# GiorgiaAuroraAdorni/gansformer-reproducibility-challenge

Hardware: NVIDIA H100
Metric: images/sec @256^2 synth (GANsformer generator forward, K=16 latents, 12 attention layers, batch 32/GPU) (higher is better)
Workload: dtype tf32 (fp32 storage; wgmma tf32 attention and stride-1 3x3 convolutions (own kernels), TF32 cuDNN up-convolutions; value_fp32_convs = the same with fp32 cuDNN convolutions)

## Files before the change

### gansformer-reproducibility-challenge_b200/_build.py

```python
from __future__ import annotations

import os
import shutil
import subprocess
from pathlib import Path

PKG_DIR = Path(__file__).resolve().parent
CSRC = PKG_DIR / "csrc"
LIB_PATH = PKG_DIR / "libgf_attn.so"
SOURCES = ["gf_api.cu", "gf_fold.cu", "gf_simt.cu", "gf_tc.cu", "gf_tc_cen.cu", "gf_tc_gemm.cu", "gf_bwd.cu", "gf_ops.cu", "gf_conv.cu"]
COMPILE_FLAGS = [
    "-gencode", "arch=compute_90a,code=sm_90a",
    "-lineinfo", "-O3", "-std=c++17",
    "-Xcompiler", "-fPIC",
]


def _nvcc() -> str:
    for cand in (os.environ.get("NVCC"), shutil.which("nvcc"), "/usr/local/cuda/bin/nvcc"):
        if cand and os.path.exists(cand):
            return cand
    raise RuntimeError("nvcc not found: cannot build libgf_attn.so (set NVCC=/path/to/nvcc)")


def _stale() -> bool:
    if not LIB_PATH.exists():
        return True
    t = LIB_PATH.stat().st_mtime
    deps = list(CSRC.glob("*.cu")) + list(CSRC.glob("*.cuh")) + list((PKG_DIR.parent / "include").glob("*.h"))
    return any(d.stat().st_mtime > t for d in deps)


def _compile_one(nvcc: str, src: Path, obj: Path, verbose: bool) -> str:
    cmd = [nvcc, *COMPILE_FLAGS, *os.environ.get("GF_NVCC_DEFS", "").split(), "-c", str(src), "-o", str(obj)]
    if verbose:
        cmd[1:1] = ["-Xptxas", "-v"]
    res = subprocess.run(cmd, capture_output=True, text=True)
    if res.returncode != 0:
        raise RuntimeError("nvcc failed:\n" + " ".join(cmd) + "\n" + res.stdout + res.stderr)
    return res.stderr


def build_extension(force: bool = False, verbose: bool = False) -> Path:
    if not force and not _stale():
        return LIB_PATH
    from concurrent.futures import ThreadPoolExecutor
    nvcc = _nvcc()
    objdir = PKG_DIR / "build"
    objdir.mkdir(exist_ok=True)
    tag = objdir / ".flags"
    flags_now = " ".join(COMPILE_FLAGS) + "|" + os.environ.get("GF_NVCC_DEFS", "")
    if not tag.exists() or tag.read_text() != flags_now:
        force = True
    hdr_time = max(d.stat().st_mtime for d in list(CSRC.glob("*.cuh")) + list((PKG_DIR.parent / "include").glob("*.h")))
    jobs = []
    for name in SOURCES:
        src, obj = CSRC / name, objdir / (name[:-3] + ".o")
        if force or verbose or not obj.exists() or obj.stat().st_mtime < max(src.stat().st_mtime, hdr_time):
            jobs.append((src, obj))
    with ThreadPoolExecutor(max_workers=min(8, max(1, len(jobs)))) as pool:
        logs = list(pool.map(lambda j: _compile_one(nvcc, j[0], j[1], verbose), jobs))
    tag.write_text(flags_now)
    cmd = [nvcc, "-gencode", "arch=compute_90a,code=sm_90a", "-shared", "-o", str(LIB_PATH)] + [str(objdir / (n[:-3] + ".o")) for n in SOURCES]
    res = subprocess.run(cmd, capture_output=True, text=True)
    if res.returncode != 0:
        raise RuntimeError("nvcc link failed:\n" + " ".join(cmd) + "\n" + res.stdout + res.stderr)
    if verbose:
        print("\n".join(logs))
    return LIB_PATH
```

### gansformer-reproducibility-challenge_b200/csrc/gf_conv.cu

```cuda
#include <stdlib.h>
#include <string.h>
#include "gf_common.cuh"
#include "gf_tc_common.cuh"
#include "../../include/gf_ops.h"

namespace gf {
namespace cv {

using namespace tc;

constexpr int PH = 8, PW = 16;
constexpr int BK = 32;
constexpr int A_ROWS = (PH + 2) * PW;
constexpr int A_BYTES = A_ROWS * BK * 4;
constexpr int NUM_THREADS = 288;
constexpr int MAX_A = 3, MAX_W = 8;

struct Bars {
  uint64_t full_a[MAX_A], empty_a[MAX_A], full_w[MAX_W], empty_w[MAX_W];
};

struct Params {
  int B, H, W, Cin, Cout;
  int tiles_h, tiles_w, tiles_n;
  long long total_tiles;
  int na, nw;
  float alpha;
};

__device__ __forceinline__ void tma_load_4d(uint32_t dst, const CUtensorMap* map, uint32_t bar, int c0, int c1, int c2, int c3) {
  asm volatile(
      "cp.async.bulk.tensor.4d.shared::cluster.global.mbarrier::complete_tx::bytes [%0], [%1, {%3, %4, %5, %6}], [%2];"
      ::"r"(dst), "l"(map), "r"(bar), "r"(c0), "r"(c1), "r"(c2), "r"(c3)
      : "memory");
}

template <int BN>
__global__ void __launch_bounds__(NUM_THREADS, 1)
conv3x3_tc_kernel(const __grid_constant__ CUtensorMap tmX, const __grid_constant__ CUtensorMap tmW, float* __restrict__ y, const Params P) {
  constexpr int W_BYTES = BN * BK * 4;
  extern __shared__ __align__(1024) uint8_t smem_raw[];
  uint8_t* smem = smem_raw + ((1024u - (smem_u32(smem_raw) & 1023u)) & 1023u);
  const uint32_t s_a = smem_u32(smem);
  const uint32_t s_w = s_a + (uint32_t)P.na * A_BYTES;
  Bars* bars = reinterpret_cast<Bars*>(smem + (size_t)P.na * A_BYTES + (size_t)P.nw * W_BYTES);
  const int warp = __shfl_sync(0xffffffffu, (int)(threadIdx.x >> 5), 0);
  const int lane = threadIdx.x & 31;

  if (warp == 8 && lane == 0) {
    prefetch_tmap(&tmX); prefetch_tmap(&tmW);
    for (int i = 0; i < P.na; ++i) { mbar_init(smem_u32(&bars->full_a[i]), 1); mbar_init(smem_u32(&bars->empty_a[i]), 2); }
    for (int i = 0; i < P.nw; ++i) { mbar_init(smem_u32(&bars->full_w[i]), 1); mbar_init(smem_u32(&bars->empty_w[i]), 2); }
    fence_barrier_init();
  }
  __syncthreads();

  auto decode = [&](long long t, int& nt, int& pw, int& ph, int& b) {
    nt = (int)(t % P.tiles_n); t /= P.tiles_n;
    pw = (int)(t % P.tiles_w); t /= P.tiles_w;
    ph = (int)(t % P.tiles_h); b = (int)(t / P.tiles_h);
  };

  if (warp == 8) {
    if (lane == 0) {
      int sa = 0, sw = 0; uint32_t pa = 0, pw_ = 0;
      for (long long t = blockIdx.x; t < P.total_tiles; t += gridDim.x) {
        int nt, pw, ph, b;
        decode(t, nt, pw, ph, b);
        const int h0 = ph * PH, w0 = pw * PW, n0 = nt * BN;
        for (int c0 = 0; c0 < P.Cin; c0 += BK) {
          for (int dx = 0; dx < 3; ++dx) {
            mbar_wait(smem_u32(&bars->empty_a[sa]), pa ^ 1u);
            const uint32_t fa = smem_u32(&bars->full_a[sa]);
            mbar_expect_tx(fa, (uint32_t)A_BYTES);
            tma_load_4d(s_a + (uint32_t)sa * A_BYTES, &tmX, fa, c0, w0 + dx - 1, h0 - 1, b);
            if (++sa == P.na) { sa = 0; pa ^= 1u; }
            for (int dy = 0; dy < 3; ++dy) {
              mbar_wait(smem_u32(&bars->empty_w[sw]), pw_ ^ 1u);
              const uint32_t fw = smem_u32(&bars->full_w[sw]);
              mbar_expect_tx(fw, (uint32_t)W_BYTES);
              tma_load_2d(s_w + (uint32_t)sw * W_BYTES, &tmW, fw, c0, (dy * 3 + dx) * P.Cout + n0);
              if (++sw == P.nw) { sw = 0; pw_ ^= 1u; }
            }
          }
        }
      }
    }
    return;
  }

  const int wg = warp >> 2;
  const int gid = lane >> 2, qd = lane & 3;
  const int rA = wg * 64 + (warp & 3) * 16 + gid;
  const bool leader = (warp & 3) == 0 && lane == 0;
  int sa = 0, sw = 0; uint32_t pa = 0, pw_ = 0;
  for (long long t = blockIdx.x; t < P.total_tiles; t += gridDim.x) {
    int nt, pw, ph, b;
    decode(t, nt, pw, ph, b);
    float acc[BN / 2];
    int prev_w = -1, prev_a = -1;
#pragma unroll 1
    for (int c0 = 0; c0 < P.Cin; c0 += BK) {
#pragma unroll 1
      for (int dx = 0; dx < 3; ++dx) {
        mbar_wait(smem_u32(&bars->full_a[sa]), pa);
        const uint32_t a_view = s_a + (uint32_t)sa * A_BYTES + wg * 64 * 128;
#pragma unroll
        for (int dy = 0; dy < 3; ++dy) {
          mbar_wait(smem_u32(&bars->full_w[sw]), pw_);
          const uint64_t da = gmma_desc(a_view + dy * PW * 128, 1024, LAYOUT_SW128);
          const uint64_t db = gmma_desc(s_w + (uint32_t)sw * W_BYTES, 1024, LAYOUT_SW128);
          const uint32_t acc0 = (c0 | dx | dy) ? 1u : 0u;
          wgmma_fence();
#pragma unroll
          for (int kk = 0; kk < 4; ++kk) wgmma_ss<BN>(acc, da + kk * 2, db + kk * 2, (acc0 | kk) ? 1u : 0u);
          wgmma_commit();
          wgmma_wait<1>();
          if (prev_w >= 0) {
            named_bar_sync(1 + wg, 128);
            if (leader) {
              mbar_arrive(smem_u32(&bars->empty_w[prev_w]));
              if (prev_a >= 0) mbar_arrive(smem_u32(&bars->empty_a[prev_a]));
            }
          }
          prev_w = sw;
          prev_a = dy == 2 ? sa : -1;
          if (++sw == P.nw) { sw = 0; pw_ ^= 1u; }
        }
        if (++sa == P.na) { sa = 0; pa ^= 1u; }
      }
    }
    wgmma_wait<0>();
    fence_regs<BN / 2>(acc);
    named_bar_sync(1 + wg, 128);
    if (leader) {
      mbar_arrive(smem_u32(&bars->empty_w[prev_w]));
      mbar_arrive(smem_u32(&bars->empty_a[prev_a]));
    }
#pragma unroll
    for (int i = 0; i < 2; ++i) {
      const int r = rA + 8 * i;
      const int h = ph * PH + (r >> 4), w = pw * PW + (r & 15);
      float* yrow = y + (((size_t)b * P.H + h) * P.W + w) * P.Cout + nt * BN + 2 * qd;
#pragma unroll
      for (int j = 0; j < BN / 8; ++j)
        *reinterpret_cast<float2*>(yrow + 8 * j) = make_float2(acc[4 * j + 2 * i] * P.alpha, acc[4 * j + 2 * i + 1] * P.alpha);
    }
  }
}

constexpr int U_PC = 16, U_PR = 8;
constexpr int U_OC = U_PC - 2;
constexpr int U_BN = 64;
constexpr int U_A_BYTES = (U_PR + 1) * U_PC * BK * 4;
constexpr int U_W_BYTES = U_BN * BK * 4;
constexpr int U_WS_BYTES = 9 * U_W_BYTES;
constexpr int U_CS = 68;
constexpr int U_NA = 4;
constexpr int U_THREADS = 384;

struct UBars {
  uint64_t full_a[U_NA], empty_a[U_NA], full_w[4], empty_w[4];
};

struct UParams {
  int B, H, W, Cin, Cout;
  int strips, steps, tiles_n;
  int total_units;
  float ag;
  const float* scale;
};

__device__ constexpr int U_GTAPS[4] = {4, 2, 2, 1};
__device__ constexpr int U_GNX[4] = {2, 2, 1, 1};
__device__ constexpr int U_GTAP[4][4] = {{8, 7, 5, 4}, {2, 1, 0, 0}, {6, 3, 0, 0}, {0, 0, 0, 0}};
__device__ constexpr int U_GOFF[4] = {0, 4, 6, 8};
__device__ constexpr int U_GROW[4] = {0, 1, 0, 1};

__device__ __forceinline__ void setmaxnreg_dec40() { asm volatile("setmaxnreg.dec.sync.aligned.u32 40;"); }
__device__ __forceinline__ void setmaxnreg_inc232() { asm volatile("setmaxnreg.inc.sync.aligned.u32 232;"); }

__global__ void __launch_bounds__(U_THREADS, 1)
upconv_blur_tc_kernel(const __grid_constant__ CUtensorMap tmX, const __grid_constant__ CUtensorMap tmW, float* __restrict__ y, const UParams P) {
  extern __shared__ __align__(1024) uint8_t smem_raw[];
  uint8_t* smem = smem_raw + ((1024u - (smem_u32(smem_raw) & 1023u)) & 1023u);
  const uint32_t s_a = smem_u32(smem);
  const uint32_t s_w = s_a + (uint32_t)U_NA * U_A_BYTES;
  float* carry = reinterpret_cast<float*>(smem + (size_t)U_NA * U_A_BYTES + U_WS_BYTES);
  float* stage = carry + 4 * 2 * U_PC * U_CS;
  UBars* bars = reinterpret_cast<UBars*>(stage + U_PR * U_PC * U_CS);
  const int warp = __shfl_sync(0xffffffffu, (int)(threadIdx.x >> 5), 0);
  const int lane = threadIdx.x & 31;

  if (warp == 8 && lane == 0) {
    prefetch_tmap(&tmX); prefetch_tmap(&tmW);
    for (int i = 0; i < U_NA; ++i) { mbar_init(smem_u32(&bars->full_a[i]), 1); mbar_init(smem_u32(&bars->empty_a[i]), 2); }
    for (int i = 0; i < 4; ++i) { mbar_init(smem_u32(&bars->full_w[i]), 1); mbar_init(smem_u32(&bars->empty_w[i]), 2); }
    fence_barrier_init();
  }
  __syncthreads();

  auto decode = [&](int u, int& nt, int& st, int& b) {
    nt = u % P.tiles_n; u /= P.tiles_n;
    st = u % P.strips; b = u / P.strips;
  };

  if (warp >= 8) {
    setmaxnreg_dec40();
    if (warp == 8 && lane == 0) {
      int sa = 0; uint32_t pa = 0, pw_ = 0;
      for (int u = blockIdx.x; u < P.total_units; u += gridDim.x) {
        int nt, st, b;
        decode(u, nt, st, b);
        const int j0 = st * U_OC, n0 = nt * U_BN;
        for (int s = 0; s < P.steps; ++s) {
          for (int c0 = 0; c0 < P.Cin; c0 += BK) {
            for (int g = 0; g < 4; ++g) {
              if (g == 0 || g == 2) {
                mbar_wait(smem_u32(&bars->empty_a[sa]), pa ^ 1u);
                const uint32_t fa = smem_u32(&bars->full_a[sa]);
                mbar_expect_tx(fa, (uint32_t)U_A_BYTES);
                tma_load_4d(s_a + (uint32_t)sa * U_A_BYTES, &tmX, fa, c0, j0 - (g == 0), s * U_PR - 1, b);
                if (++sa == U_NA) { sa = 0; pa ^= 1u; }
              }
              mbar_wait(smem_u32(&bars->empty_w[g]), pw_ ^ 1u);
              const uint32_t fw = smem_u32(&bars->full_w[g]);
              mbar_expect_tx(fw, (uint32_t)(U_GTAPS[g] * U_W_BYTES));
              for (int k = 0; k < U_GTAPS[g]; ++k)
                tma_load_2d(s_w + (uint32_t)(U_GOFF[g] + k) * U_W_BYTES, &tmW, fw, c0, U_GTAP[g][k] * P.Cout + n0);
            }
            pw_ ^= 1u;
          }
        }
      }
    }
    return;
  }

  setmaxnreg_inc232();
  const int wg = warp >> 2;
  const int gid = lane >> 2, qd = lane & 3;
  const bool leader = (warp & 3) == 0 && lane == 0;
  const int cp = lane & 7, cg = lane >> 3;
  int sa = 0; uint32_t pa = 0, pw_ = 0;
  for (int u = blockIdx.x; u < P.total_units; u += gridDim.x) {
    int nt, st, b;
    decode(u, nt, st, b);
    const int j0 = st * U_OC, n0 = nt * U_BN;
    for (int s = 0; s < P.steps; ++s) {
      float accx[U_BN], accy[U_BN];
      int prev_a = -1;
      uint32_t a_view = 0;
#pragma unroll 1
      for (int c0 = 0; c0 < P.Cin; c0 += BK) {
#pragma unroll
        for (int g = 0; g < 4; ++g) {
          if (g == 0 || g == 2) {
            mbar_wait(smem_u32(&bars->full_a[sa]), pa);
            a_view = s_a + (uint32_t)sa * U_A_BYTES + wg * 4 * U_PC * 128;
          }
          mbar_wait(smem_u32(&bars->full_w[g]), pw_);
          const uint64_t da = gmma_desc(a_view + U_GROW[g] * U_PC * 128, 1024, LAYOUT_SW128);
          const uint64_t db = gmma_desc(s_w + (uint32_t)U_GOFF[g] * U_W_BYTES, 1024, LAYOUT_SW128);
          const uint64_t dby = db + (uint64_t)(U_GNX[g] * U_W_BYTES >> 4);
          const int ny = U_GTAPS[g] - U_GNX[g];
          const uint32_t acc0 = (c0 > 0 || g > 0) ? 1u : 0u;
          wgmma_fence();
#pragma unroll
          for (int kk = 0; kk < 4; ++kk) {
            const uint32_t ac = (acc0 | kk) ? 1u : 0u;
            if (U_GNX[g] == 2) wgmma_ss<128>(accx, da + kk * 2, db + kk * 2, ac);
            else wgmma_ss<64>(accx, da + kk * 2, db + kk * 2, ac);
            if (ny == 2) wgmma_ss<128>(accy, da + kk * 2, dby + kk * 2, ac);
            else if (ny == 1) wgmma_ss<64>(accy, da + kk * 2, dby + kk * 2, ac);
          }
          wgmma_commit();
          wgmma_wait<1>();
          if (c0 > 0 || g > 0) {
            named_bar_sync(1 + wg, 128);
            if (leader) {
              mbar_arrive(smem_u32(&bars->empty_w[(g + 3) & 3]));
              if (prev_a >= 0) mbar_arrive(smem_u32(&bars->empty_a[prev_a]));
            }
          }
          prev_a = (g == 1 || g == 3) ? sa : -1;
          if (g == 1 || g == 3) { if (++sa == U_NA) { sa = 0; pa ^= 1u; } }
        }
        pw_ ^= 1u;
      }
      wgmma_wait<0>();
      fence_regs<U_BN>(accx);
      fence_regs<U_BN>(accy);
      named_bar_sync(1 + wg, 128);
      if (leader) {
        mbar_arrive(smem_u32(&bars->empty_w[3]));
        mbar_arrive(smem_u32(&bars->empty_a[prev_a]));
      }

      const int io = s * U_PR - 2 + warp;
#pragma unroll
      for (int sl = 0; sl < U_BN / 16; ++sl) {
        float* my_row = stage + warp * U_PC * U_CS;
#pragma unroll
        for (int ph = 0; ph < 4; ++ph)
#pragma unroll
          for (int jj = 0; jj < 2; ++jj)
#pragma unroll
            for (int i = 0; i < 2; ++i)
              *reinterpret_cast<float2*>(my_row + (gid + 8 * i) * U_CS + ph * 16 + jj * 8 + 2 * qd) =
                  make_float2((ph < 2 ? accx : accy)[32 * (ph & 1) + 4 * (2 * sl + jj) + 2 * i], (ph < 2 ? accx : accy)[32 * (ph & 1) + 4 * (2 * sl + jj) + 2 * i + 1]);
        named_bar_sync(3, 256);
        if (io >= 0 && io < P.H) {
          auto row = [&](int r) -> const float* {
            return (r < 2 ? carry + (sl * 2 + r) * U_PC * U_CS : stage + (r - 2) * U_PC * U_CS) + 2 * cp;
          };
          const int ch = n0 + sl * 16 + 2 * cp;
          const float2 d = __ldg(reinterpret_cast<const float2*>(P.scale + (size_t)b * P.Cout + ch));
          const float2 f = make_float2(P.ag * d.x, P.ag * d.y);
          const int Wo = 2 * P.W;
#pragma unroll 1
          for (int p = cg; p < U_OC && j0 + p < P.W; p += 4) {
            float* y0 = y + (((size_t)b * 2 * P.H + 2 * io) * Wo + 2 * (j0 + p)) * P.Cout + ch;
            float2 e0, o0, e1, o1;
#pragma unroll
            for (int v = 0; v < 5; ++v) {
              const float* base = row(warp + v / 2) + ((v & 1) ? 0 : 32) + p * U_CS;
              const float2 E0 = *reinterpret_cast<const float2*>(base), O0 = *reinterpret_cast<const float2*>(base + 16);
              const float2 E1 = *reinterpret_cast<const float2*>(base + U_CS), O1 = *reinterpret_cast<const float2*>(base + U_CS + 16);
              const float2 O2 = *reinterpret_cast<const float2*>(base + 2 * U_CS + 16);
              float2 h0, h1;
              h0.x = ((O0.x + 3.f * E0.x) + 3.f * O1.x) + E1.x;
              h0.y = ((O0.y + 3.f * E0.y) + 3.f * O1.y) + E1.y;
              h1.x = ((E0.x + 3.f * O1.x) + 3.f * E1.x) + O2.x;
              h1.y = ((E0.y + 3.f * O1.y) + 3.f * E1.y) + O2.y;
              if (v == 0) { e0 = h0; e1 = h1; }
              else if (v == 1) {
                e0.x += 3.f * h0.x; e0.y += 3.f * h0.y; o0 = h0;
                e1.x += 3.f * h1.x; e1.y += 3.f * h1.y; o1 = h1;
              } else if (v == 2) {
                e0.x += 3.f * h0.x; e0.y += 3.f * h0.y; o0.x += 3.f * h0.x; o0.y += 3.f * h0.y;
                e1.x += 3.f * h1.x; e1.y += 3.f * h1.y; o1.x += 3.f * h1.x; o1.y += 3.f * h1.y;
              } else if (v == 3) {
                e0.x += h0.x; e0.y += h0.y; o0.x += 3.f * h0.x; o0.y += 3.f * h0.y;
                e1.x += h1.x; e1.y += h1.y; o1.x += 3.f * h1.x; o1.y += 3.f * h1.y;
              } else {
                o0.x += h0.x; o0.y += h0.y;
                o1.x += h1.x; o1.y += h1.y;
              }
            }
            *reinterpret_cast<float2*>(y0) = make_float2(e0.x * 0.015625f * f.x, e0.y * 0.015625f * f.y);
            *reinterpret_cast<float2*>(y0 + P.Cout) = make_float2(e1.x * 0.015625f * f.x, e1.y * 0.015625f * f.y);
            *reinterpret_cast<float2*>(y0 + (size_t)Wo * P.Cout) = make_float2(o0.x * 0.015625f * f.x, o0.y * 0.015625f * f.y);
            *reinterpret_cast<float2*>(y0 + (size_t)Wo * P.Cout + P.Cout) = make_float2(o1.x * 0.015625f * f.x, o1.y * 0.015625f * f.y);
          }
        }
        named_bar_sync(3, 256);
        if (warp >= U_PR - 2) {
          float* crow = carry + (sl * 2 + warp - (U_PR - 2)) * U_PC * U_CS;
#pragma unroll
          for (int ph = 0; ph < 4; ++ph)
#pragma unroll
            for (int jj = 0; jj < 2; ++jj)
#pragma unroll
              for (int i = 0; i < 2; ++i)
                *reinterpret_cast<float2*>(crow + (gid + 8 * i) * U_CS + ph * 16 + jj * 8 + 2 * qd) =
                    make_float2((ph < 2 ? accx : accy)[32 * (ph & 1) + 4 * (2 * sl + jj) + 2 * i], (ph < 2 ? accx : accy)[32 * (ph & 1) + 4 * (2 * sl + jj) + 2 * i + 1]);
        }
      }
    }
  }
}

static int make_map_nhwc(CUtensorMap* m, const void* base, int B, int H, int W, int C, int box_c, int box_w, int box_h) {
  EncodeTiledFn enc = get_encode();
  if (!enc) { set_error("cuTensorMapEncodeTiled entry point not available"); return GF_ERR_CUDA; }
  cuuint64_t dims[4] = {(cuuint64_t)C, (cuuint64_t)W, (cuuint64_t)H, (cuuint64_t)B};
  cuuint64_t strides[3] = {(cuuint64_t)C * 4, (cuuint64_t)W * C * 4, (cuuint64_t)H * W * C * 4};
  cuuint32_t box[4] = {(cuuint32_t)box_c, (cuuint32_t)box_w, (cuuint32_t)box_h, 1};
  cuuint32_t estr[4] = {1, 1, 1, 1};
  CUresult r = enc(m, CU_TENSOR_MAP_DATA_TYPE_FLOAT32, 4, const_cast<void*>(base), dims, strides, box, estr, CU_TENSOR_MAP_INTERLEAVE_NONE,
                   CU_TENSOR_MAP_SWIZZLE_128B, CU_TENSOR_MAP_L2_PROMOTION_L2_128B, CU_TENSOR_MAP_FLOAT_OOB_FILL_NONE);
  if (r != CUDA_SUCCESS) { set_error("cuTensorMapEncodeTiled (NHWC 4-D) failed with CUresult %d (B=%d H=%d W=%d C=%d)", (int)r, B, H, W, C); return GF_ERR_CUDA; }
  return GF_OK;
}

template <int BN>
static int launch_bn(const float* x, const float* wt, float* y, int B, int H, int W, int Cin, int Cout, cudaStream_t st) {
  constexpr int W_BYTES = BN * BK * 4;
  CUtensorMap tmX, tmW;
  int rc;
  if ((rc = make_map_nhwc(&tmX, x, B, H, W, Cin, BK, PW, PH + 2))) return rc;
  if ((rc = make_map(&tmW, wt, (uint64_t)9 * Cout, (uint64_t)Cin, BN, BK, CU_TENSOR_MAP_SWIZZLE_128B))) return rc;
  Params P;
  P.B = B; P.H = H; P.W = W; P.Cin = Cin; P.Cout = Cout;
  P.tiles_h = H / PH; P.tiles_w = W / PW; P.tiles_n = Cout / BN;
  P.total_tiles = (long long)B * P.tiles_h * P.tiles_w * P.tiles_n;
  const int avail = device_smem_optin() - (int)sizeof(Bars) - 1024;
  P.na = MAX_A;
  P.nw = (avail - P.na * A_BYTES) / W_BYTES;
  if (P.nw > MAX_W) P.nw = MAX_W;
  if (P.nw < 2) { set_error("conv3x3: shared memory too small"); return GF_ERR_UNSUPPORTED; }
  P.alpha = 1.000352220f;
  const int smem_bytes = P.na * A_BYTES + P.nw * W_BYTES + (int)sizeof(Bars) + 1024;
  GF_CUDA_OK(cudaFuncSetAttribute(conv3x3_tc_kernel<BN>, cudaFuncAttributeMaxDynamicSharedMemorySize, smem_bytes));
  long long grid = device_sms();
  if (grid > P.total_tiles) grid = P.total_tiles;
  conv3x3_tc_kernel<BN><<<(unsigned)grid, NUM_THREADS, smem_bytes, st>>>(tmX, tmW, y, P);
  GF_LAUNCH_OK();
  return GF_OK;
}

static int launch(const float* x, const float* wt, float* y, int B, int H, int W, int Cin, int Cout, cudaStream_t st) {
  if (Cout % 256 == 0) return launch_bn<256>(x, wt, y, B, H, W, Cin, Cout, st);
  if (Cout % 128 == 0) return launch_bn<128>(x, wt, y, B, H, W, Cin, Cout, st);
  return launch_bn<64>(x, wt, y, B, H, W, Cin, Cout, st);
}

static int launch_upconv(const float* x, const float* wt, const float* scale, float* y, int B, int H, int W, int Cin, int Cout,
                         float gain, cudaStream_t st) {
  CUtensorMap tmX, tmW;
  int rc;
  if ((rc = make_map_nhwc(&tmX, x, B, H, W, Cin, BK, U_PC, U_PR + 1))) return rc;
  if ((rc = make_map(&tmW, wt, (uint64_t)9 * Cout, (uint64_t)Cin, U_BN, BK, CU_TENSOR_MAP_SWIZZLE_128B))) return rc;
  UParams P;
  P.B = B; P.H = H; P.W = W; P.Cin = Cin; P.Cout = Cout;
  P.strips = (W + U_OC - 1) / U_OC;
  P.steps = (H + 2 + U_PR - 1) / U_PR;
  P.tiles_n = Cout / U_BN;
  const long long units = (long long)B * P.strips * P.tiles_n;
  if (units > (1ll << 30)) { set_error("upconv3x3_blur: too many work units (%lld)", units); return GF_ERR_UNSUPPORTED; }
  P.total_units = (int)units;
  P.ag = 1.000352220f * gain;
  P.scale = scale;
  const int smem_bytes = U_NA * U_A_BYTES + U_WS_BYTES + 8 * U_PC * U_CS * 4 + U_PR * U_PC * U_CS * 4 + (int)sizeof(UBars) + 1024;
  if (smem_bytes > device_smem_optin()) { set_error("upconv3x3_blur: shared memory too small"); return GF_ERR_UNSUPPORTED; }
  GF_CUDA_OK(cudaFuncSetAttribute(upconv_blur_tc_kernel, cudaFuncAttributeMaxDynamicSharedMemorySize, smem_bytes));
  long long grid = device_sms();
  if (grid > P.total_units) grid = P.total_units;
  upconv_blur_tc_kernel<<<(unsigned)grid, U_THREADS, smem_bytes, st>>>(tmX, tmW, y, P);
  GF_LAUNCH_OK();
  return GF_OK;
}

__global__ void pack_weights_kernel(const float* __restrict__ w, float* __restrict__ wt, int Cout, int Cin, float scale) {
  const size_t total = (size_t)9 * Cout * Cin;
  for (size_t i = blockIdx.x * (size_t)blockDim.x + threadIdx.x; i < total; i += (size_t)gridDim.x * blockDim.x) {
    const int ci = (int)(i % Cin);
    const int o = (int)((i / Cin) % Cout);
    const int tap = (int)(i / ((size_t)Cin * Cout));
    wt[i] = round_tf32_rn(w[((size_t)o * Cin + ci) * 9 + tap] * scale);
  }
}

}
}

using namespace gf;

extern "C" int gf_conv3x3_pack_weights(const float* w, float* wt, int Cout, int Cin, float scale, void* stream) {
  if (!w || !wt || Cout <= 0 || Cin <= 0) { set_error("gf_conv3x3_pack_weights: bad arguments"); return GF_ERR_INVALID; }
  const size_t total = (size_t)9 * Cout * Cin;
  size_t blocks = (total + 255) / 256;
  if (blocks > (size_t)num_sms() * 16) blocks = (size_t)num_sms() * 16;
  cv::pack_weights_kernel<<<(unsigned)blocks, 256, 0, (cudaStream_t)stream>>>(w, wt, Cout, Cin, scale);
  GF_LAUNCH_OK();
  return GF_OK;
}

extern "C" int gf_conv3x3_nhwc_tf32(const float* x, const float* wt, float* y, int B, int H, int W, int Cin, int Cout, void* stream) {
  if (!x || !wt || !y) { set_error("gf_conv3x3_nhwc_tf32: null pointer"); return GF_ERR_INVALID; }
  if (B <= 0 || H <= 0 || W <= 0 || H % cv::PH || W % cv::PW || Cin % cv::BK || Cout % 64 || Cin <= 0 || Cout <= 0) {
    set_error("gf_conv3x3_nhwc_tf32: needs positive sizes, H %% 8 == 0, W %% 16 == 0, Cin %% 32 == 0, Cout %% 64 == 0 (got B=%d H=%d W=%d Cin=%d Cout=%d)", B, H, W, Cin, Cout);
    return GF_ERR_UNSUPPORTED;
  }
  if (((uintptr_t)x & 15) || ((uintptr_t)wt & 15) || ((uintptr_t)y & 15)) { set_error("gf_conv3x3_nhwc_tf32: pointers must be 16-byte aligned"); return GF_ERR_INVALID; }
  int rc;
  if ((rc = check_device())) return rc;
  return cv::launch(x, wt, y, B, H, W, Cin, Cout, (cudaStream_t)stream);
}

extern "C" int gf_upconv3x3_blur_nhwc_tf32(const float* x, const float* wt, const float* scale, float* y, int B, int H, int W, int Cin,
                                           int Cout, float gain, void* stream) {
  if (!x || !wt || !scale || !y) { set_error("gf_upconv3x3_blur_nhwc_tf32: null pointer"); return GF_ERR_INVALID; }
  if (B <= 0 || H <= 0 || W <= 0 || Cin <= 0 || Cout <= 0 || Cin % cv::BK || Cout % cv::U_BN) {
    set_error("gf_upconv3x3_blur_nhwc_tf32: needs positive sizes, Cin %% 32 == 0, Cout %% 64 == 0 (got B=%d H=%d W=%d Cin=%d Cout=%d)", B, H, W, Cin, Cout);
    return GF_ERR_UNSUPPORTED;
  }
  if (((uintptr_t)x & 15) || ((uintptr_t)wt & 15) || ((uintptr_t)y & 15) || ((uintptr_t)scale & 15)) {
    set_error("gf_upconv3x3_blur_nhwc_tf32: pointers must be 16-byte aligned"); return GF_ERR_INVALID;
  }
  int rc;
  if ((rc = check_device())) return rc;
  return cv::launch_upconv(x, wt, scale, y, B, H, W, Cin, Cout, gain, (cudaStream_t)stream);
}
```

Measured before the change: 2287.

## Move upconv horizontal blur into registers via warp shuffles before staging

The horizontal half of the blur filter in the fused upconv+blur kernel now runs on the accumulator registers using warp shuffles, before results are staged to shared memory. The epilogue then reads pre-blurred values instead of reloading five neighbours and recombining them. The staging row stride changes from 68 to 72 to alter the bank mapping, and the store-loop bound is made compile-time so it can be unrolled. Optional clock64-based profiling hooks and build variants are added behind a define, so they are inactive by default.

```diff
diff --git a/gansformer-reproducibility-challenge_b200/_build.py b/gansformer-reproducibility-challenge_b200/_build.py
--- a/gansformer-reproducibility-challenge_b200/_build.py
+++ b/gansformer-reproducibility-challenge_b200/_build.py
@@ -23,16 +23,16 @@
     raise RuntimeError("nvcc not found: cannot build libgf_attn.so (set NVCC=/path/to/nvcc)")
 
 
-def _stale() -> bool:
-    if not LIB_PATH.exists():
+def _stale(lib_path: Path = LIB_PATH) -> bool:
+    if not lib_path.exists():
         return True
-    t = LIB_PATH.stat().st_mtime
+    t = lib_path.stat().st_mtime
     deps = list(CSRC.glob("*.cu")) + list(CSRC.glob("*.cuh")) + list((PKG_DIR.parent / "include").glob("*.h"))
     return any(d.stat().st_mtime > t for d in deps)
 
 
-def _compile_one(nvcc: str, src: Path, obj: Path, verbose: bool) -> str:
-    cmd = [nvcc, *COMPILE_FLAGS, *os.environ.get("GF_NVCC_DEFS", "").split(), "-c", str(src), "-o", str(obj)]
+def _compile_one(nvcc: str, src: Path, obj: Path, verbose: bool, defs: tuple = ()) -> str:
+    cmd = [nvcc, *COMPILE_FLAGS, *os.environ.get("GF_NVCC_DEFS", "").split(), *defs, "-c", str(src), "-o", str(obj)]
     if verbose:
         cmd[1:1] = ["-Xptxas", "-v"]
     res = subprocess.run(cmd, capture_output=True, text=True)
@@ -41,15 +41,16 @@
     return res.stderr
 
 
-def build_extension(force: bool = False, verbose: bool = False) -> Path:
-    if not force and not _stale():
-        return LIB_PATH
+def build_extension(force: bool = False, verbose: bool = False, variant: str = "", defs: tuple = ()) -> Path:
+    lib_path = PKG_DIR / f"libgf_attn_{variant}.so" if variant else LIB_PATH
+    if not force and not _stale(lib_path):
+        return lib_path
     from concurrent.futures import ThreadPoolExecutor
     nvcc = _nvcc()
-    objdir = PKG_DIR / "build"
-    objdir.mkdir(exist_ok=True)
+    objdir = PKG_DIR / "build" / variant if variant else PKG_DIR / "build"
+    objdir.mkdir(parents=True, exist_ok=True)
     tag = objdir / ".flags"
-    flags_now = " ".join(COMPILE_FLAGS) + "|" + os.environ.get("GF_NVCC_DEFS", "")
+    flags_now = " ".join(COMPILE_FLAGS) + "|" + os.environ.get("GF_NVCC_DEFS", "") + "|" + " ".join(defs)
     if not tag.exists() or tag.read_text() != flags_now:
         force = True
     hdr_time = max(d.stat().st_mtime for d in list(CSRC.glob("*.cuh")) + list((PKG_DIR.parent / "include").glob("*.h")))
@@ -59,12 +60,12 @@
         if force or verbose or not obj.exists() or obj.stat().st_mtime < max(src.stat().st_mtime, hdr_time):
             jobs.append((src, obj))
     with ThreadPoolExecutor(max_workers=min(8, max(1, len(jobs)))) as pool:
-        logs = list(pool.map(lambda j: _compile_one(nvcc, j[0], j[1], verbose), jobs))
+        logs = list(pool.map(lambda j: _compile_one(nvcc, j[0], j[1], verbose, tuple(defs)), jobs))
     tag.write_text(flags_now)
-    cmd = [nvcc, "-gencode", "arch=compute_90a,code=sm_90a", "-shared", "-o", str(LIB_PATH)] + [str(objdir / (n[:-3] + ".o")) for n in SOURCES]
+    cmd = [nvcc, "-gencode", "arch=compute_90a,code=sm_90a", "-shared", "-o", str(lib_path)] + [str(objdir / (n[:-3] + ".o")) for n in SOURCES]
     res = subprocess.run(cmd, capture_output=True, text=True)
     if res.returncode != 0:
         raise RuntimeError("nvcc link failed:\n" + " ".join(cmd) + "\n" + res.stdout + res.stderr)
     if verbose:
         print("\n".join(logs))
-    return LIB_PATH
+    return lib_path
diff --git a/gansformer-reproducibility-challenge_b200/csrc/gf_conv.cu b/gansformer-reproducibility-challenge_b200/csrc/gf_conv.cu
--- a/gansformer-reproducibility-challenge_b200/csrc/gf_conv.cu
+++ b/gansformer-reproducibility-challenge_b200/csrc/gf_conv.cu
@@ -155,7 +155,7 @@
 constexpr int U_A_BYTES = (U_PR + 1) * U_PC * BK * 4;
 constexpr int U_W_BYTES = U_BN * BK * 4;
 constexpr int U_WS_BYTES = 9 * U_W_BYTES;
-constexpr int U_CS = 68;
+constexpr int U_CS = 72;
 constexpr int U_NA = 4;
 constexpr int U_THREADS = 384;
 
@@ -179,6 +179,20 @@
 
 __device__ __forceinline__ void setmaxnreg_dec40() { asm volatile("setmaxnreg.dec.sync.aligned.u32 40;"); }
 __device__ __forceinline__ void setmaxnreg_inc232() { asm volatile("setmaxnreg.inc.sync.aligned.u32 232;"); }
+
+enum { UPROF_FULL_W, UPROF_FULL_A, UPROF_MMA, UPROF_EPI, UPROF_EMPTY_W, UPROF_EMPTY_A, UPROF_CONS, UPROF_PROD, UPROF_N };
+#ifdef GF_UPCONV_PROFILE
+__device__ unsigned long long g_uprof[UPROF_N];
+#define UPROF(...) __VA_ARGS__
+#else
+#define UPROF(...)
+#endif
+#define UPROF_WAIT(bar, parity, acc)                                  \
+  do {                                                               \
+    UPROF(const long long t_w0_ = clock64();)                        \
+    mbar_wait(bar, parity);                                          \
+    UPROF(acc += clock64() - t_w0_;)                                 \
+  } while (0)
 
 __global__ void __launch_bounds__(U_THREADS, 1)
 upconv_blur_tc_kernel(const __grid_constant__ CUtensorMap tmX, const __grid_constant__ CUtensorMap tmW, float* __restrict__ y, const UParams P) {
@@ -191,6 +205,7 @@
   UBars* bars = reinterpret_cast<UBars*>(stage + U_PR * U_PC * U_CS);
   const int warp = __shfl_sync(0xffffffffu, (int)(threadIdx.x >> 5), 0);
   const int lane = threadIdx.x & 31;
+  UPROF(const long long t_start = clock64(); long long pr[UPROF_N] = {};)
 
   if (warp == 8 && lane == 0) {
     prefetch_tmap(&tmX); prefetch_tmap(&tmW);
@@ -217,13 +232,13 @@
           for (int c0 = 0; c0 < P.Cin; c0 += BK) {
             for (int g = 0; g < 4; ++g) {
               if (g == 0 || g == 2) {
-                mbar_wait(smem_u32(&bars->empty_a[sa]), pa ^ 1u);
+                UPROF_WAIT(smem_u32(&bars->empty_a[sa]), pa ^ 1u, pr[UPROF_EMPTY_A]);
                 const uint32_t fa = smem_u32(&bars->full_a[sa]);
                 mbar_expect_tx(fa, (uint32_t)U_A_BYTES);
                 tma_load_4d(s_a + (uint32_t)sa * U_A_BYTES, &tmX, fa, c0, j0 - (g == 0), s * U_PR - 1, b);
                 if (++sa == U_NA) { sa = 0; pa ^= 1u; }
               }
-              mbar_wait(smem_u32(&bars->empty_w[g]), pw_ ^ 1u);
+              UPROF_WAIT(smem_u32(&bars->empty_w[g]), pw_ ^ 1u, pr[UPROF_EMPTY_W]);
               const uint32_t fw = smem_u32(&bars->full_w[g]);
               mbar_expect_tx(fw, (uint32_t)(U_GTAPS[g] * U_W_BYTES));
               for (int k = 0; k < U_GTAPS[g]; ++k)
@@ -233,6 +248,8 @@
           }
         }
       }
+      UPROF(pr[UPROF_PROD] = clock64() - t_start;
+            for (int i = 0; i < UPROF_N; ++i) if (pr[i]) atomicAdd(&g_uprof[i], (unsigned long long)pr[i]);)
     }
     return;
   }
@@ -241,7 +258,8 @@
   const int wg = warp >> 2;
   const int gid = lane >> 2, qd = lane & 3;
   const bool leader = (warp & 3) == 0 && lane == 0;
-  const int cp = lane & 7, cg = lane >> 3;
+  const int cp = (lane & 3) | (lane >> 4) << 2, cg = (lane >> 2) & 3;
+  const int src1 = (lane + 4) & 31, src2 = (lane + 8) & 31;
   int sa = 0; uint32_t pa = 0, pw_ = 0;
   for (int u = blockIdx.x; u < P.total_units; u += gridDim.x) {
     int nt, st, b;
@@ -251,15 +269,16 @@
       float accx[U_BN], accy[U_BN];
       int prev_a = -1;
       uint32_t a_view = 0;
+      UPROF(const long long t_mma = clock64();)
 #pragma unroll 1
       for (int c0 = 0; c0 < P.Cin; c0 += BK) {
 #pragma unroll
         for (int g = 0; g < 4; ++g) {
           if (g == 0 || g == 2) {
-            mbar_wait(smem_u32(&bars->full_a[sa]), pa);
+            UPROF_WAIT(smem_u32(&bars->full_a[sa]), pa, pr[UPROF_FULL_A]);
             a_view = s_a + (uint32_t)sa * U_A_BYTES + wg * 4 * U_PC * 128;
           }
-          mbar_wait(smem_u32(&bars->full_w[g]), pw_);
+          UPROF_WAIT(smem_u32(&bars->full_w[g]), pw_, pr[UPROF_FULL_W]);
           const uint64_t da = gmma_desc(a_view + U_GROW[g] * U_PC * 128, 1024, LAYOUT_SW128);
           const uint64_t db = gmma_desc(s_w + (uint32_t)U_GOFF[g] * U_W_BYTES, 1024, LAYOUT_SW128);
           const uint64_t dby = db + (uint64_t)(U_GNX[g] * U_W_BYTES >> 4);
@@ -291,11 +310,32 @@
       wgmma_wait<0>();
       fence_regs<U_BN>(accx);
       fence_regs<U_BN>(accy);
+      UPROF(const long long t_epi = clock64(); pr[UPROF_MMA] += t_epi - t_mma;)
       named_bar_sync(1 + wg, 128);
       if (leader) {
         mbar_arrive(smem_u32(&bars->empty_w[3]));
         mbar_arrive(smem_u32(&bars->empty_a[prev_a]));
       }
+
+      auto hblur = [&](float (&a)[U_BN]) {
+#pragma unroll
+        for (int j = 0; j < 8; ++j)
+#pragma unroll
+          for (int e = 0; e < 2; ++e) {
+            const int ie = 4 * j + e, iO = 32 + 4 * j + e;
+            const float Ea = a[ie], Eb = a[ie + 2], Oa = a[iO], Ob = a[iO + 2];
+            const float sEa = __shfl_sync(0xffffffffu, Ea, src1), sEb = __shfl_sync(0xffffffffu, Eb, src1);
+            const float sOa = __shfl_sync(0xffffffffu, Oa, src1), sOb = __shfl_sync(0xffffffffu, Ob, src1);
+            const float tOa = __shfl_sync(0xffffffffu, Oa, src2), tOb = __shfl_sync(0xffffffffu, Ob, src2);
+            const float E1a = gid < 7 ? sEa : sEb, O1a = gid < 7 ? sOa : sOb, O2a = gid < 6 ? tOa : tOb;
+            a[ie] = ((Oa + 3.f * Ea) + 3.f * O1a) + E1a;
+            a[iO] = ((Ea + 3.f * O1a) + 3.f * E1a) + O2a;
+            a[ie + 2] = ((Ob + 3.f * Eb) + 3.f * sOb) + sEb;
+            a[iO + 2] = ((Eb + 3.f * sOb) + 3.f * sEb) + tOb;
+          }
+      };
+      hblur(accx);
+      hblur(accy);
 
       const int io = s * U_PR - 2 + warp;
 #pragma unroll
@@ -318,21 +358,14 @@
           const float2 d = __ldg(reinterpret_cast<const float2*>(P.scale + (size_t)b * P.Cout + ch));
           const float2 f = make_float2(P.ag * d.x, P.ag * d.y);
           const int Wo = 2 * P.W;
-#pragma unroll 1
-          for (int p = cg; p < U_OC && j0 + p < P.W; p += 4) {
+#pragma unroll
+          for (int p = cg; p < U_OC; p += 4) {
             float* y0 = y + (((size_t)b * 2 * P.H + 2 * io) * Wo + 2 * (j0 + p)) * P.Cout + ch;
             float2 e0, o0, e1, o1;
 #pragma unroll
             for (int v = 0; v < 5; ++v) {
               const float* base = row(warp + v / 2) + ((v & 1) ? 0 : 32) + p * U_CS;
-              const float2 E0 = *reinterpret_cast<const float2*>(base), O0 = *reinterpret_cast<const float2*>(base + 16);
-              const float2 E1 = *reinterpret_cast<const float2*>(base + U_CS), O1 = *reinterpret_cast<const float2*>(base + U_CS + 16);
-              const float2 O2 = *reinterpret_cast<const float2*>(base + 2 * U_CS + 16);
-              float2 h0, h1;
-              h0.x = ((O0.x + 3.f * E0.x) + 3.f * O1.x) + E1.x;
-              h0.y = ((O0.y + 3.f * E0.y) + 3.f * O1.y) + E1.y;
-              h1.x = ((E0.x + 3.f * O1.x) + 3.f * E1.x) + O2.x;
-              h1.y = ((E0.y + 3.f * O1.y) + 3.f * E1.y) + O2.y;
+              const float2 h0 = *reinterpret_cast<const float2*>(base), h1 = *reinterpret_cast<const float2*>(base + 16);
               if (v == 0) { e0 = h0; e1 = h1; }
               else if (v == 1) {
                 e0.x += 3.f * h0.x; e0.y += 3.f * h0.y; o0 = h0;
@@ -348,6 +381,7 @@
                 o1.x += h1.x; o1.y += h1.y;
               }
             }
+            if (j0 + p >= P.W) continue;
             *reinterpret_cast<float2*>(y0) = make_float2(e0.x * 0.015625f * f.x, e0.y * 0.015625f * f.y);
             *reinterpret_cast<float2*>(y0 + P.Cout) = make_float2(e1.x * 0.015625f * f.x, e1.y * 0.015625f * f.y);
             *reinterpret_cast<float2*>(y0 + (size_t)Wo * P.Cout) = make_float2(o0.x * 0.015625f * f.x, o0.y * 0.015625f * f.y);
@@ -367,8 +401,13 @@
                     make_float2((ph < 2 ? accx : accy)[32 * (ph & 1) + 4 * (2 * sl + jj) + 2 * i], (ph < 2 ? accx : accy)[32 * (ph & 1) + 4 * (2 * sl + jj) + 2 * i + 1]);
         }
       }
+      UPROF(pr[UPROF_EPI] += clock64() - t_epi;)
     }
   }
+  UPROF(if ((warp & 3) == 0 && lane == 0) {
+          pr[UPROF_CONS] = clock64() - t_start;
+          for (int i = 0; i < UPROF_N; ++i) if (pr[i]) atomicAdd(&g_uprof[i], (unsigned long long)pr[i]);
+        })
 }
 
 static int make_map_nhwc(CUtensorMap* m, const void* base, int B, int H, int W, int C, int box_c, int box_w, int box_h) {
@@ -493,3 +532,13 @@
   if ((rc = check_device())) return rc;
   return cv::launch_upconv(x, wt, scale, y, B, H, W, Cin, Cout, gain, (cudaStream_t)stream);
 }
+
+#ifdef GF_UPCONV_PROFILE
+extern "C" int gf_upconv_profile_read(unsigned long long* out) {
+  GF_CUDA_OK(cudaDeviceSynchronize());
+  GF_CUDA_OK(cudaMemcpyFromSymbol(out, cv::g_uprof, sizeof(cv::g_uprof)));
+  const unsigned long long zero[cv::UPROF_N] = {};
+  GF_CUDA_OK(cudaMemcpyToSymbol(cv::g_uprof, zero, sizeof(zero)));
+  return GF_OK;
+}
+#endif
```

Result: faster. 2329, median of 6 (+1.8%).
